# HazyResearch/hyena-dna

Measured on AMD Instinct MI355X. Metric: nucleotides/sec fwd+bwd at L=1M d=256; fftconv achieved HBM GB/s vs peak, higher is better.
Workload: dtype f32

## Files before the change

hyena_dna_amd/_lib.py:

```python
import ctypes
import os
import threading

import torch

HERE = os.path.dirname(os.path.abspath(__file__))
LIB_PATH = os.path.join(HERE, "csrc", "libhyena_fftconv.so")
ABI_VERSION = 3

HYENA_F32, HYENA_BF16, HYENA_F16 = 0, 1, 2
MAX_L = 1048576
PLAN_NONE, PLAN_ONCHIP, PLAN_TWO_LEVEL = 0, 1, 2

_DTYPES = {torch.float32: HYENA_F32, torch.bfloat16: HYENA_BF16, torch.float16: HYENA_F16}

_lock = threading.Lock()
_lib = None
_tables = {}
_workspace = {}


class HyenaLibraryError(RuntimeError):
    pass

# ... 110 lines not shown
                                        c_void_p]
        L.hyena_cm_post_bwd.restype = c_int
        L.hyena_cm_post_bwd.argtypes = [c_void_p, c_void_p, c_void_p, c_void_p, c_void_p, c_void_p, c_void_p, c_void_p, c_void_p,
                                        c_int, c_int, c_int, c_int, c_int, c_void_p]
        L.hyena_cm_pre_bwd.restype = c_int
        L.hyena_cm_pre_bwd.argtypes = [c_void_p, c_void_p, c_void_p, c_void_p, c_void_p, c_void_p, c_void_p,
                                       c_int, c_int, c_int, c_int, c_int, c_void_p]
        L.hyena_cm_pre_fwd_ld.restype = c_int
        L.hyena_cm_pre_fwd_ld.argtypes = [c_void_p, c_void_p, c_void_p, c_void_p, c_void_p, c_int, c_int, c_int, c_int, ctypes.c_long, c_int, c_int,
                                          c_int, c_void_p]
        L.hyena_cm_post_fwd_ld.restype = c_int
        L.hyena_cm_post_fwd_ld.argtypes = [c_void_p, c_void_p, c_void_p, c_void_p, c_void_p, c_void_p, c_int, c_int, c_int, c_int, ctypes.c_long, c_int,
                                           ctypes.c_long, c_int, c_int, c_int, c_void_p]
        L.hyena_cm_post_bwd_ld.restype = c_int
        L.hyena_cm_post_bwd_ld.argtypes = [c_void_p, c_void_p, c_void_p, c_void_p, c_void_p, c_void_p, c_void_p, c_void_p, c_void_p,
                                           c_int, c_int, c_int, c_int, ctypes.c_long, c_int, ctypes.c_long, c_int, c_int, c_int, c_void_p]
        L.hyena_cm_pre_bwd_ld.restype = c_int
        L.hyena_cm_pre_bwd_ld.argtypes = [c_void_p, c_void_p, c_void_p, c_void_p, c_void_p, c_void_p, c_void_p,
                                          c_int, c_int, c_int, c_int, ctypes.c_long, c_int, c_int, c_int, c_void_p]
        L.hyena_decode_partial_floats.restype = c_size_t
        L.hyena_decode_partial_floats.argtypes = [c_int, c_int, c_int]
        L.hyena_decode_pre.restype = c_int
        L.hyena_decode_pre.argtypes = [c_void_p, c_int, c_void_p, c_void_p, c_void_p, c_void_p, c_void_p, c_void_p, c_void_p,
                                       c_int, c_int, c_int, c_int, c_int, c_int, c_void_p]
        L.hyena_decode_conv.restype = c_int
        L.hyena_decode_conv.argtypes = [c_void_p, c_int, c_void_p, c_void_p, c_void_p, c_int, c_int, c_int, c_int, c_int, c_void_p]
        L.hyena_decode_post.restype = c_int
        L.hyena_decode_post.argtypes = [c_void_p, c_void_p, c_void_p, c_void_p, c_void_p, c_void_p, c_int, c_int, c_int, c_int, c_int, c_void_p]
        for rows, one in ((L.hyena_decode_pre_rows, L.hyena_decode_pre), (L.hyena_decode_conv_rows, L.hyena_decode_conv),
                          (L.hyena_decode_post_rows, L.hyena_decode_post)):
            rows.restype, rows.argtypes = c_int, one.argtypes
        L.hyena_decode_pre_fan.restype = c_int
        L.hyena_decode_pre_fan.argtypes = [c_void_p, c_int, c_void_p, c_void_p, c_void_p, c_void_p, c_void_p, c_void_p, c_void_p,
                                           c_int, c_int, c_int, c_int, c_int, c_int, c_int, c_void_p]
        L.hyena_decode_conv_fan.restype = c_int
        L.hyena_decode_conv_fan.argtypes = [c_void_p, c_int, c_void_p, c_void_p, c_void_p, c_void_p, c_int, c_int, c_int, c_int, c_int, c_int,
                                            c_int, c_int, c_void_p]
        L.hyena_decode_post_fan.restype = c_int
        L.hyena_decode_post_fan.argtypes = [c_void_p, c_void_p, c_void_p, c_void_p, c_void_p, c_void_p, c_int, c_int, c_int, c_int, c_int, c_int,
                                            c_int, c_void_p]
        L.hyena_decode_block_partial_floats.restype = c_size_t
        L.hyena_decode_block_partial_floats.argtypes = [c_int, c_int, c_int, c_int]
        for blk, one in ((L.hyena_decode_pre_block, L.hyena_decode_pre), (L.hyena_decode_conv_block, L.hyena_decode_conv),
                         (L.hyena_decode_post_block, L.hyena_decode_post), (L.hyena_decode_pre_block_fan, L.hyena_decode_pre_fan),
                         (L.hyena_decode_conv_block_fan, L.hyena_decode_conv_fan), (L.hyena_decode_post_block_fan, L.hyena_decode_post_fan)):
            blk.restype, blk.argtypes = c_int, one.argtypes[:-1] + [c_int, c_void_p]
        L.hyena_decode_sample.restype = c_int
        L.hyena_decode_sample.argtypes = [c_void_p, ctypes.c_long, c_int, c_int, c_int, c_int, ctypes.c_float, c_int, ctypes.c_float, c_void_p,
                                          c_int, c_int, c_void_p, c_void_p, c_void_p, ctypes.c_long, c_int, c_void_p, ctypes.c_long,
                                          c_void_p, c_void_p, c_void_p]
        L.hyena_inproj_pre_fwd_ld.restype = c_int
        L.hyena_inproj_pre_fwd_ld.argtypes = [c_void_p, c_void_p, c_void_p, c_void_p, c_void_p, c_void_p, c_void_p,
                                              c_int, c_int, c_int, c_int, ctypes.c_long, c_int, c_int, c_int, c_void_p]
        L.hyena_outproj_gate_addnorm_fwd_ld.restype = c_int
        L.hyena_outproj_gate_addnorm_fwd_ld.argtypes = [c_void_p, c_void_p, c_void_p, c_void_p, c_void_p, c_void_p, c_void_p, c_void_p, c_void_p,
                                                        c_void_p, ctypes.c_float, c_void_p, c_void_p, c_void_p, c_void_p, c_void_p,
                                                        c_int, c_int, c_int, c_int, ctypes.c_long, c_int, ctypes.c_long, c_int, c_int, c_int,
                                                        c_void_p]
        L.hyena_outproj_dgrad_supported.restype = c_int
        L.hyena_outproj_dgrad_supported.argtypes = [c_int, c_int, c_int, c_int]
        L.hyena_outproj_dgrad_partial_floats.restype = c_size_t
        L.hyena_outproj_dgrad_partial_floats.argtypes = [c_int, c_int, c_int]
        L.hyena_outproj_dgrad_gate_bwd_ld.restype = c_int
        L.hyena_outproj_dgrad_gate_bwd_ld.argtypes = [c_void_p, c_void_p, c_void_p, c_void_p, c_void_p, c_void_p, c_void_p, c_void_p, c_void_p,
                                                      c_void_p, c_int, c_int, c_int, c_int, ctypes.c_long, c_int, c_int, c_int, c_void_p]
        L.hyena_outproj_gate_fwd_ld.restype = c_int
        L.hyena_outproj_gate_fwd_ld.argtypes = [c_void_p, c_void_p, c_void_p, c_void_p, c_void_p, c_void_p, c_void_p, c_void_p, c_void_p,
                                                c_int, c_int, c_int, c_int, ctypes.c_long, c_int, ctypes.c_long, c_int, c_int, c_int, c_void_p]
        L.hyena_proj_supported.restype = c_int
        L.hyena_proj_supported.argtypes = [c_int, c_int, c_int, c_int]
        L.hyena_inproj_pre_fwd.restype = c_int
        L.hyena_inproj_pre_fwd.argtypes = [c_void_p, c_void_p, c_void_p, c_void_p, c_void_p, c_void_p, c_void_p,
                                           c_int, c_int, c_int, c_int, c_int, c_void_p]
        L.hyena_outproj_supported.restype = c_int
        L.hyena_outproj_supported.argtypes = [c_int, c_int, c_int, c_int]
        L.hyena_proj_kernel_generation.restype = c_int
        L.hyena_proj_kernel_generation.argtypes = [c_int, c_int]
        gen = os.environ.get("HYENA_OUTPROJ_KERNEL")
        if gen in ("1", "2"):
            L.hyena_proj_kernel_generation(0, int(gen))
        gen = os.environ.get("HYENA_INPROJ_KERNEL")
        if gen in ("1", "2"):
            L.hyena_proj_kernel_generation(1, int(gen))
        L.hyena_outproj_gate_fwd.restype = c_int
        L.hyena_outproj_gate_fwd.argtypes = [c_void_p, c_void_p, c_void_p, c_void_p, c_void_p, c_void_p, c_void_p, c_void_p, c_void_p,
                                             c_int, c_int, c_int, c_int, c_int, c_void_p]
        L.hyena_colsum_supported.restype = c_int
        L.hyena_colsum_supported.argtypes = [ctypes.c_long, c_int, c_int]
        L.hyena_colsum_partial_floats.restype = c_size_t
        L.hyena_colsum_partial_floats.argtypes = [ctypes.c_long, c_int]
        L.hyena_colsum.restype = c_int
        L.hyena_colsum.argtypes = [c_void_p, c_void_p, c_void_p, ctypes.c_long, c_int, c_int, c_void_p]
        L.hyena_mlp_supported.restype = c_int
        L.hyena_mlp_supported.argtypes = [ctypes.c_long, c_int, c_int, c_int]
        L.hyena_mlp_partial_floats.restype = c_size_t
        L.hyena_mlp_partial_floats.argtypes = [ctypes.c_long, c_int]
        L.hyena_mlp_fc1_gelu_fwd.restype = c_int
        L.hyena_mlp_fc1_gelu_fwd.argtypes = [c_void_p, c_void_p, c_void_p, c_void_p, c_void_p, ctypes.c_long, c_int, c_int, c_int, c_void_p]
        L.hyena_mlp_dh_dgelu_bwd.restype = c_int
        L.hyena_mlp_dh_dgelu_bwd.argtypes = [c_void_p, c_void_p, c_void_p, c_void_p, c_void_p, ctypes.c_long, c_int, c_int, c_int, c_void_p]
        L.hyena_filter_supported.restype = c_int
        L.hyena_filter_supported.argtypes = [c_int, c_int, c_int, c_int]
        L.hyena_filter_saved_bytes.restype = c_size_t
        L.hyena_filter_saved_bytes.argtypes = [c_int]
        L.hyena_filter_workspace_bytes.restype = c_size_t
        L.hyena_filter_workspace_bytes.argtypes = [c_int, c_int]
        L.hyena_filter_fwd.restype = c_int
        L.hyena_filter_fwd.argtypes = [ctypes.POINTER(FilterParams), c_void_p, c_void_p, c_void_p]
        L.hyena_filter_bwd.restype = c_int
        L.hyena_filter_bwd.argtypes = [ctypes.POINTER(FilterParams), c_void_p, c_void_p, ctypes.POINTER(FilterGrads),
                                       c_void_p, c_size_t, c_void_p]
        L.hyena_filter16_saved_bytes.restype = c_size_t
        L.hyena_filter16_saved_bytes.argtypes = [c_int]
        L.hyena_filter16_fwd.restype = c_int
        L.hyena_filter16_fwd.argtypes = [ctypes.POINTER(FilterParams), c_int, c_void_p, c_void_p, c_void_p]
        L.hyena_filter16_bwd.restype = c_int
        L.hyena_filter16_bwd.argtypes = [ctypes.POINTER(FilterParams), c_int, c_void_p, c_void_p, ctypes.POINTER(FilterGrads),
                                         c_void_p, c_size_t, c_void_p]
        L.hyena_filter_row_pitch.restype = c_int
        L.hyena_filter_row_pitch.argtypes = [c_int]
        L.hyena_filter_fwd_ld.restype = c_int
        L.hyena_filter_fwd_ld.argtypes = [ctypes.POINTER(FilterParams), c_void_p, c_int, c_void_p, c_void_p]
        L.hyena_filter_bwd_ld.restype = c_int
        L.hyena_filter_bwd_ld.argtypes = [ctypes.POINTER(FilterParams), c_void_p, c_int, c_void_p, ctypes.POINTER(FilterGrads),
                                          c_void_p, c_size_t, c_void_p]
        L.hyena_filter16_fwd_ld.restype = c_int
        L.hyena_filter16_fwd_ld.argtypes = [ctypes.POINTER(FilterParams), c_int, c_void_p, c_int, c_void_p, c_void_p]
        L.hyena_filter16_bwd_ld.restype = c_int
        L.hyena_filter16_bwd_ld.argtypes = [ctypes.POINTER(FilterParams), c_int, c_void_p, c_int, c_void_p, ctypes.POINTER(FilterGrads),
                                            c_void_p, c_size_t, c_void_p]
        c_long, c_float = ctypes.c_long, ctypes.c_float
        L.hyena_add_norm_supported.restype = c_int
        L.hyena_add_norm_supported.argtypes = [c_int, c_int, c_int]
        L.hyena_add_norm_fwd.restype = c_int
        L.hyena_add_norm_fwd.argtypes = [c_void_p, c_int, c_void_p, c_void_p, c_void_p, c_float, c_void_p, c_int, c_void_p,
                                         c_void_p, c_void_p, c_long, c_int, c_void_p]
        L.hyena_dropout_add_norm_fwd.restype = c_int
        L.hyena_dropout_add_norm_fwd.argtypes = [c_void_p, c_int, c_void_p, c_void_p, c_void_p, c_float, c_float, c_void_p, c_void_p, c_int,
                                                 c_void_p, c_void_p, c_void_p, c_long, c_int, c_void_p]
        L.hyena_dropout_add_norm_bwd.restype = c_int
        L.hyena_dropout_add_norm_bwd.argtypes = [c_void_p, c_int, c_void_p, c_void_p, c_void_p, c_void_p, c_void_p, c_float, c_void_p,
                                                 c_void_p, c_int, c_void_p, c_void_p, c_void_p, c_void_p, c_long, c_int, c_void_p]
        L.hyena_dropout_add_norm_bwd_colsum.restype = c_int
        L.hyena_dropout_add_norm_bwd_colsum.argtypes = [c_void_p, c_int, c_void_p, c_void_p, c_void_p, c_void_p, c_void_p, c_float, c_void_p,
                                                        c_void_p, c_int, c_void_p, c_void_p, c_void_p, c_void_p, c_void_p, c_long, c_int, c_void_p]
        L.hyena_embed_add_norm_supported.restype = c_int
        L.hyena_embed_add_norm_supported.argtypes = [c_int, c_int, c_int]
        L.hyena_embed_add_norm_fwd.restype = c_int
        L.hyena_embed_add_norm_fwd.argtypes = [c_void_p, c_void_p, c_int, c_void_p, c_void_p, c_float, c_float, c_void_p, c_void_p, c_int,
                                               c_void_p, c_void_p, c_void_p, c_long, c_int, c_void_p]
        L.hyena_embed_add_norm_partial_floats.restype = c_size_t
        L.hyena_embed_add_norm_partial_floats.argtypes = [c_long, c_int]
        L.hyena_embed_add_norm_bwd.restype = c_int
        L.hyena_embed_add_norm_bwd.argtypes = [c_void_p, c_int, c_void_p, c_void_p, c_void_p, c_void_p, c_void_p, c_void_p, c_float, c_void_p,
                                               c_void_p, c_int, c_void_p, c_void_p, c_void_p, c_long, c_int, c_void_p]
        L.hyena_add_norm_partial_floats.restype = c_size_t
        L.hyena_add_norm_partial_floats.argtypes = [c_long, c_int]
        L.hyena_add_norm_bwd.restype = c_int
        L.hyena_add_norm_bwd.argtypes = [c_void_p, c_int, c_void_p, c_void_p, c_void_p, c_void_p, c_void_p, c_void_p, c_int,
                                         c_void_p, c_void_p, c_void_p, c_void_p, c_long, c_int, c_void_p]
        L.hyena_add_norm_pool_supported.restype = c_int
        L.hyena_add_norm_pool_supported.argtypes = [c_int, c_int]
        L.hyena_add_norm_pool_partial_floats.restype = c_size_t
        L.hyena_add_norm_pool_partial_floats.argtypes = [c_int, c_long, c_int]
        L.hyena_add_norm_pool_fwd.restype = c_int
        L.hyena_add_norm_pool_fwd.argtypes = [c_void_p, c_int, c_void_p, c_void_p, c_void_p, c_float, c_float, c_void_p, c_void_p, c_int,
# ... 977 lines not shown
```

hyena_dna_amd/csrc/proj.hip:

```cpp
#include "proj_kernels.h"
#include "proj2_kernels.h"
#include "launch.h"
#include <type_traits>
#include "../../include/hyena_fftconv.h"
#include "../../include/hyena_proj.h"

using namespace hyena;

namespace {
template <auto Kernel, class Args>
int pj_launch(size_t lds, int threads, int grid, void* stream, const Args& a) {
    static thread_local int done = -1;
    hy_allow_lds(Kernel, lds, &done);
    HY_LAUNCH(Kernel, dim3(grid), dim3(threads), lds, stream, a);
    return hy_launch_error() ? HYENA_ERR_LAUNCH : HYENA_OK;
}
bool pj_kd_ok(int K, int dtype) { return (K == 128 || K == 256) && (dtype == HYENA_BF16 || dtype == HYENA_F16); }
template <class F>
int pj_dispatch(int K, int dtype, F f) {
    typedef std::integral_constant<int, DT_BF16> BF;
    typedef std::integral_constant<int, DT_F16> HF;
    if (K == 256) return dtype == HYENA_BF16 ? f(std::integral_constant<int, 256>(), BF()) : f(std::integral_constant<int, 256>(), HF());
    return dtype == HYENA_BF16 ? f(std::integral_constant<int, 128>(), BF()) : f(std::integral_constant<int, 128>(), HF());
}
int pj_runs(int tiles, int cap, int min_run, int* tiles_per_wg) {
    const int runs = cap < tiles ? cap : tiles;
    int len = (tiles + runs - 1) / runs;
    if (len < min_run && tiles >= min_run) len = min_run;
    *tiles_per_wg = len;
    return (tiles + len - 1) / len;
}
int pj_grid(int runs, int ncg) { return ((runs + 7) / 8) * 8 * ncg; }

void mlp_schedule(size_t P, int ncg, pj::MlpArgs* a, int* runs_out, int* grid_out) {
    a->tiles = (int)((P + pj::PJ_NT - 1) / pj::PJ_NT);
    *runs_out = pj_runs(a->tiles, 256 * 8 / ncg, 8, &a->tiles_per_wg);
    *grid_out = pj_grid(*runs_out, ncg);
}
void dgrad_schedule(int B, int L, int D, pj::DgArgs* a, int* runs_out, int* grid_out) {
    const int ncg = D / (pj::PJ_WAVES * pj::DG_CB);
    a->tiles_per_seq = (L + pj::PJ_NT - 1) / pj::PJ_NT;
    a->tiles = B * a->tiles_per_seq;
    a->nrec = *runs_out = pj_runs(a->tiles, 256 * DG_WGS / ncg, 16, &a->tiles_per_wg);
    *grid_out = pj_grid(*runs_out, ncg);
}
template <int MODE>
int dispatch_mlp(const pj::MlpArgs& a, int K, int dtype, int grid, void* stream) {
    return pj_dispatch(K, dtype, [&](auto k, auto dt) {
        constexpr int KK = decltype(k)::value, DT = decltype(dt)::value;
        return pj_launch<pj::mlp_kernel<KK, DT, MODE>>(pj::PmCfg<KK>::lds(MODE), pj::PJ_THREADS, grid, stream, a);
    });
}
int g_outproj_generation = 2;
int g_inproj_generation = 1;
}

#if defined(PJ_PROFILE)
extern "C" int hyena_pj_prof_set(void* buf) {
    return (int)hipMemcpyToSymbol(HIP_SYMBOL(hyena::pj::pj_prof_buf), &buf, sizeof(buf));
}
#endif

extern "C" {

static int colsum_groups(long P) {
    long g = (P + 511) / 512;
    return (int)(g < 1 ? 1 : (g > 512 ? 512 : g));
}

int hyena_colsum_supported(long P, int N, int dtype) {
    if (!(dtype == HYENA_BF16 || dtype == HYENA_F16) || N < 8 || N % 8 != 0 || pj::PJ_THREADS % (N / 8) != 0) return 0;
    return P >= 1 && (size_t)P < ((size_t)1 << 31) ? 1 : 0;
}

size_t hyena_colsum_partial_floats(long P, int N) { return P < 1 || N < 1 ? 0 : (size_t)colsum_groups(P) * N; }

int hyena_colsum(const void* x, float* part, float* out, long P, int N, int dtype, void* stream) {
    if (x == nullptr || part == nullptr || out == nullptr || !hyena_colsum_supported(P, N, dtype)) return HYENA_ERR_BAD_ARG;
    pj::ColsumArgs a;
    a.x = x; a.part = part; a.out = out; a.P = (unsigned)P; a.N = N; a.G = colsum_groups(P);
    a.rows_per_wg = (int)((P + a.G - 1) / a.G);
    a.G = (int)((P + a.rows_per_wg - 1) / a.rows_per_wg);
    const size_t lds = (size_t)pj::PJ_THREADS * 8 * sizeof(float);
    if (dtype == HYENA_BF16) HY_LAUNCH((pj::colsum_kernel<DT_BF16>), dim3(a.G), dim3(pj::PJ_THREADS), lds, stream, a);
    else HY_LAUNCH((pj::colsum_kernel<DT_F16>), dim3(a.G), dim3(pj::PJ_THREADS), lds, stream, a);
    HY_LAUNCH(pj::colsum_final_kernel, dim3((N + 63) / 64), dim3(pj::PJ_THREADS), pj::PJ_THREADS * sizeof(float), stream, a);
    return hy_launch_error() ? HYENA_ERR_LAUNCH : HYENA_OK;
}

int hyena_mlp_supported(long P, int K, int N, int dtype) {
    if (!pj_kd_ok(K, dtype)) return 0;
    if (N < 256 || N % 256 != 0 || P < 1) return 0;
    return (size_t)P < ((size_t)1 << 31) ? 1 : 0;
}

size_t hyena_mlp_partial_floats(long P, int N) {
    if (P < 1 || N < 256) return 0;
    pj::MlpArgs a;
    int runs, grid;
    mlp_schedule((size_t)P, N / 256, &a, &runs, &grid);
    return (size_t)runs * N;
}

int hyena_mlp_fc1_gelu_fwd(const void* x, const void* W1, const float* b1, void* a_out, void* h_out, long P, int K, int N, int dtype,
                           void* stream) {
    if (x == nullptr || W1 == nullptr || a_out == nullptr || h_out == nullptr || !hyena_mlp_supported(P, K, N, dtype)) return HYENA_ERR_BAD_ARG;
    pj::MlpArgs a;
    a.x = x; a.W = W1; a.bias = b1; a.a_in = nullptr; a.o0 = a_out; a.o1 = h_out; a.part = nullptr; a.P = (unsigned)P; a.N = N;
    int runs, grid;
    mlp_schedule((size_t)P, N / 256, &a, &runs, &grid);
    return dispatch_mlp<0>(a, K, dtype, grid, stream);
}

int hyena_mlp_dh_dgelu_bwd(const void* dy, const void* W2T, const void* a_in, void* da, float* part, long P, int K, int N, int dtype,
                           void* stream) {
    if (dy == nullptr || W2T == nullptr || a_in == nullptr || da == nullptr || part == nullptr || !hyena_mlp_supported(P, K, N, dtype))
        return HYENA_ERR_BAD_ARG;
    pj::MlpArgs a;
    a.x = dy; a.W = W2T; a.bias = nullptr; a.a_in = a_in; a.o0 = da; a.o1 = nullptr; a.part = part; a.P = (unsigned)P; a.N = N;
    int runs, grid;
    mlp_schedule((size_t)P, N / 256, &a, &runs, &grid);
    return dispatch_mlp<1>(a, K, dtype, grid, stream);
}

int hyena_proj_kernel_generation(int family, int generation) {
    if (family != 0 && family != 1) return -1;
    int& g = family == 0 ? g_outproj_generation : g_inproj_generation;
    if (generation == 1 || generation == 2) g = generation;
    else if (generation > 0) return -1;
    return g;
}

int hyena_outproj_supported(int B, int L, int D, int dtype) {
    if (!pj_kd_ok(D, dtype)) return 0;
    if (B < 1 || L < 64) return 0;
    return (size_t)B * (size_t)L < ((size_t)1 << 31) ? 1 : 0;
}

int hyena_outproj_gate_fwd(const void* y, const void* xT, const float* bin, const float* w, const float* b, const void* W,
                           const float* bias, void* out, void* zT, int B, int L, int Lx, int D, int dtype, void* stream) {
    return hyena_outproj_gate_fwd_ld(y, xT, bin, w, b, W, bias, out, zT, B, L, Lx, D, (long)B * Lx, Lx, (long)B * L, L, L, dtype, stream);
}

int hyena_outproj_gate_fwd_ld(const void* y, const void* xT, const float* bin, const float* w, const float* b, const void* W,
                              const float* bias, void* out, void* zT, int B, int L, int Lx, int D, long csx, int bsx, long csz, int bsz,
                              int lda, int dtype, void* stream) {
    return hyena_outproj_gate_addnorm_fwd_ld(y, xT, bin, w, b, W, bias, nullptr, nullptr, nullptr, 0.f, out, nullptr, nullptr, nullptr, zT, B, L,
                                             Lx, D, csx, bsx, csz, bsz, lda, dtype, stream);
}

static bool pj_layout_ok(long cs, int bs, int B, int len) { return bs >= len && cs >= (long)(B - 1) * bs + len; }

int hyena_outproj_gate_addnorm_fwd_ld(const void* y, const void* xT, const float* bin, const float* w, const float* b, const void* W,
                                      const float* bias, const float* residual_in, const float* ln_weight, const float* ln_bias, float eps,
                                      void* out, float* residual_out, float* mean, float* rstd, void* zT, int B, int L, int Lx, int D,
                                      long csx, int bsx, long csz, int bsz, int lda, int dtype, void* stream) {
    if (y == nullptr || xT == nullptr || w == nullptr || b == nullptr || W == nullptr || out == nullptr || L > Lx || lda < L ||
        !hyena_outproj_supported(B, L, D, dtype) || !pj_layout_ok(csx, bsx, B, Lx) || (zT != nullptr && !pj_layout_ok(csz, bsz, B, L)))
        return HYENA_ERR_BAD_ARG;
    if (ln_weight != nullptr && (ln_bias == nullptr || residual_out == nullptr || mean == nullptr || rstd == nullptr ||
                                 residual_out == residual_in))
        return HYENA_ERR_BAD_ARG;
    pj::OutProjArgs a;
    a.y = y; a.xT = xT; a.bin = bin; a.w = w; a.b = b; a.W = W; a.bias = bias; a.out = out; a.zT = zT;
    a.res_in = residual_in; a.ln_w = ln_weight; a.ln_b = ln_bias; a.res_out = residual_out; a.mean = mean; a.rstd = rstd; a.eps = eps;
    a.B = B; a.L = L; a.Lx = Lx; a.D = D; a.csx = csx; a.bsx = bsx; a.csz = csz; a.bsz = bsz; a.lda = lda;
    a.tiles_per_seq = (L + pj::PJ_NT - 1) / pj::PJ_NT;
    a.tiles = B * a.tiles_per_seq;
    const bool gen2 = g_outproj_generation == 2;
    const bool ln = ln_weight != nullptr;
    const int runs = pj_runs(a.tiles, 256 * (gen2 && D == 256 ? 4 : 8), 8, &a.tiles_per_wg);
    return pj_dispatch(D, dtype, [&](auto k, auto dt) {
        constexpr int K = decltype(k)::value, DT = decltype(dt)::value;
        typedef pj::Op2Cfg<K> C2;
        typedef pj::OpCfg<K> C1;
        if (gen2)
            return ln ? pj_launch<pj::outproj_gate_fwd2_kernel<K, DT, true>>(C2::LDS_LN, C2::THREADS, runs, stream, a)
                      : pj_launch<pj::outproj_gate_fwd2_kernel<K, DT, false>>(C2::LDS, C2::THREADS, runs, stream, a);
        return ln ? pj_launch<pj::outproj_gate_fwd_kernel<K, DT, true>>(C1::LDS_LN, pj::PJ_THREADS, runs, stream, a)
                  : pj_launch<pj::outproj_gate_fwd_kernel<K, DT, false>>(C1::LDS, pj::PJ_THREADS, runs, stream, a);
    });
}

int hyena_outproj_dgrad_supported(int B, int L, int D, int dtype) {
    if (!pj_kd_ok(D, dtype)) return 0;
    if (B < 1 || L < 1) return 0;
    return (size_t)B * (size_t)L < ((size_t)1 << 31) - 64 ? 1 : 0;
}

size_t hyena_outproj_dgrad_partial_floats(int B, int L, int D) {
    if (B < 1 || L < 1 || !(D == 128 || D == 256)) return 0;
    pj::DgArgs a;
    int runs, grid;
    dgrad_schedule(B, L, D, &a, &runs, &grid);
    return (size_t)D * runs * 8;
}

int hyena_outproj_dgrad_gate_bwd_ld(const void* dy, const void* Wt, const void* y, const void* xT, const float* bin, const float* w,
                                    const float* b, void* dyc, void* dxT, float* part, int B, int L, int Lx, int D, long csx, int bsx,
                                    int lda, int dtype, void* stream) {
    if (dy == nullptr || Wt == nullptr || y == nullptr || xT == nullptr || w == nullptr || b == nullptr || dyc == nullptr || dxT == nullptr ||
        part == nullptr || L > Lx || !pj_layout_ok(csx, bsx, B, Lx) || lda < L || !hyena_outproj_dgrad_supported(B, L, D, dtype))
        return HYENA_ERR_BAD_ARG;
    pj::DgArgs a;
    a.dy = dy; a.Wt = Wt; a.y = y; a.xT = xT; a.bin = bin; a.w = w; a.b = b; a.dyc = dyc; a.dxT = dxT; a.part = part;
    a.B = B; a.L = L; a.Lx = Lx; a.D = D; a.csx = csx; a.bsx = bsx; a.lda = lda;
    int runs, grid;
    dgrad_schedule(B, L, D, &a, &runs, &grid);
    return pj_dispatch(D, dtype, [&](auto k, auto dt) {
        constexpr int K = decltype(k)::value, DT = decltype(dt)::value;
// ... 49 lines not shown
```

hyena_dna_amd/csrc/proj2_kernels.h:

```cpp
#pragma once
#include "proj_kernels.h"

namespace hyena {
namespace pj {

template <int K> struct Op2Cfg {
    static_assert(K == 128 || K == 256, "d_model of the HyenaDNA models");
    static constexpr int WAVES = K / 16;
    static constexpr int THREADS = WAVES * 64;
    static constexpr int KS = K / 32;
    static constexpr int RND = K / (WAVES * 8);
    static constexpr int ZBUF = PJ_NT * K * 2;
    static constexpr int TAPB = K * 8 * 4;
    static constexpr int OROW = (K + 8) * 2;
    static constexpr int OBUF = PJ_NT * OROW;
    static constexpr int ROWS = PJ_NT / WAVES;
    static constexpr size_t LDS = (size_t)ZBUF + TAPB + OBUF;
    static constexpr int RROW = K * 4;
    static constexpr int RBUF = PJ_NT * RROW;
    static constexpr size_t LDS_LN = LDS + RBUF;
};

template <int K, int DT, bool LN>
__global__ void __launch_bounds__(Op2Cfg<K>::THREADS, 4) outproj_gate_fwd2_kernel(OutProjArgs a) {
// ... 456 lines not shown
                vg_half(0, 0, prod);
                vg_half(0, 1, prod);
                vg_store(0, prod);
            } else {
                product(0, Q);
                HY_SCHED_FENCE();
                xt_load();
                HY_SCHED_FENCE();
                product(Q, 2 * Q);
                HY_SCHED_FENCE();
                xt_store(0, 2);
                HY_SCHED_FENCE();
                product(2 * Q, 3 * Q);
                HY_SCHED_FENCE();
                xt_store(2, 4);
                HY_SCHED_FENCE();
                product(3 * Q, 4 * Q);
                HY_SCHED_FENCE();
                vg_half(0, 0, prod);
                HY_SCHED_FENCE();
                product(4 * Q, 5 * Q);
                HY_SCHED_FENCE();
                vg_half(0, 1, prod);
                vg_store(0, prod);
                HY_SCHED_FENCE();
                product(5 * Q, 6 * Q);
                HY_SCHED_FENCE();
                if (nunits > 1) vg_half(1, 0, prod);
                HY_SCHED_FENCE();
                product(6 * Q, 7 * Q);
                HY_SCHED_FENCE();
                if (nunits > 1) { vg_half(1, 1, prod); vg_store(1, prod); }
                HY_SCHED_FENCE();
                product(7 * Q, C::KS);
            }
        } else {
            if (pend) row_phase_generic();
            product(0, C::KS);
        }
        PJ_MARK(3);
        PJ_BARRIER();
        PJ_MARK(4);
        if (have) {
            if (lane < IP2_CB) {
                HY_LDS uint32_t* row = reinterpret_cast<HY_LDS uint32_t*>(et + (lr0 + lane) * C::EROW);
                row[3] = row[3 + PJ_NT / 2];
            }
            HY_WAVE_SYNC_PJ();
            HY_UNROLL
            for (int pt = 0; pt < 2; ++pt) {
                elem_t e16[16];
                HY_UNROLL
                for (int r = 0; r < 16; ++r) e16[r] = Elem<DT>::cvt(acc[pt][r]);
                Frag f0, f1;
                __builtin_memcpy(f0.w, e16, 16);
                __builtin_memcpy(f1.w, e16 + 8, 16);
                HY_LDS char* dst = et + (lr0 + j) * C::EROW + (8 + 32 * pt + 16 * hb) * 2;
                lds_st16(dst, f0);
                lds_st16(dst + 16, f1);
            }
        }
        pend = have && t >= t_begin;
        pend_fast = p0 + PJ_NT <= P && sl0 >= 2 && sl0 + PJ_NT <= a.Lc;
        prev_p0 = p0; prev_sb = sb; prev_sl0 = sl0;
        PJ_MARK(5);
    }
#if defined(PJ_PROFILE) && !defined(HIPEMU)
    asm volatile("s_waitcnt vmcnt(0)" ::: "memory");
    PJ_MARK(9);
    asm volatile("s_memrealtime %0\n\ts_waitcnt lgkmcnt(0)" : "=s"(pj_rt1)::"memory");
    if (pj_prof_buf != nullptr && lane == 0) {
        unsigned long long* o = pj_prof_buf + ((size_t)blockIdx.x * IP2_WAVES + wave) * 16;
        HY_UNROLL
        for (int i = 0; i < 10; ++i) o[i] = pj_d[i];
        o[10] = (unsigned long long)(t_end - t_first + 1);
        o[11] = pj_t - pj_start;
        o[12] = pj_rt1 - pj_rt0;
    }
#endif
}

}
}
```

hyena_dna_amd/csrc/proj_kernels.h:

```cpp
#pragma once
#define HY_HELPERS_ONLY
#include "fftconv_kernels.h"
#include "block_kernels.h"

namespace hyena {
namespace pj {

enum { PJ_THREADS = 256, PJ_WAVES = 4, PJ_NT = 64 ,
       PJ_EW = PJ_NT + 8  };

#ifdef HIPEMU
#define HY_WAVE_SYNC_PJ() hipemu::yield(2)
#else
#define HY_WAVE_SYNC_PJ() __builtin_amdgcn_wave_barrier()
#endif

#if defined(PJ_PROFILE) && !defined(HIPEMU)
__device__ unsigned long long* pj_prof_buf = nullptr;
#define PJ_NOW(v)                                                                                       \
    do {                                                                                                \
        __builtin_amdgcn_sched_barrier(0);                                                              \
        asm volatile("s_memtime %0\n\ts_waitcnt lgkmcnt(0)" : "=s"(v)::"memory");                       \
        __builtin_amdgcn_sched_barrier(0);                                                              \
    } while (0)
// ... 24 lines not shown
        return __builtin_amdgcn_mfma_f32_32x32x16_f16(__builtin_bit_cast(v8, a), __builtin_bit_cast(v8, b), c, 0, 0, 0);
    }
}
#endif

#ifdef HIPEMU
__device__ __forceinline__ Frag ld16(const void* p) { Frag f; __builtin_memcpy(f.w, p, 16); return f; }
__device__ __forceinline__ void st16(void* p, const Frag& f) { __builtin_memcpy(p, f.w, 16); }
__device__ __forceinline__ Frag lds_ld16(const HY_LDS char* p) { return ld16(p); }
__device__ __forceinline__ void lds_st16(HY_LDS char* p, const Frag& f) { st16(p, f); }
#else
typedef unsigned pj_vec16 __attribute__((ext_vector_type(4), aligned(2)));
typedef unsigned pj_lvec16 __attribute__((ext_vector_type(4)));
__device__ __forceinline__ Frag ld16(const void* p) {
#ifdef PJ_DBG_NO_LD
    Frag f; f.w[0] = f.w[1] = f.w[2] = f.w[3] = (uint32_t)(size_t)p; return f;
#else
    return __builtin_bit_cast(Frag, *reinterpret_cast<const pj_vec16*>(p));
#endif
}
#ifndef PJ_POL_ST
#define PJ_POL_ST 1
#endif
__device__ __forceinline__ void st16(void* p, const Frag& f) {
#ifdef PJ_DBG_NO_ST
    if (f.w[0] == 0x12345678u && f.w[3] == 0x9abcdef0u) *reinterpret_cast<pj_vec16*>(p) = __builtin_bit_cast(pj_vec16, f);
#else
    if (PJ_POL_ST) __builtin_nontemporal_store(__builtin_bit_cast(pj_vec16, f), reinterpret_cast<pj_vec16*>(p));
    else *reinterpret_cast<pj_vec16*>(p) = __builtin_bit_cast(pj_vec16, f);
#endif
}
__device__ __forceinline__ Frag lds_ld16(const HY_LDS char* p) { return __builtin_bit_cast(Frag, *reinterpret_cast<const HY_LDS pj_lvec16*>(p)); }
__device__ __forceinline__ void lds_st16(HY_LDS char* p, const Frag& f) { *reinterpret_cast<HY_LDS pj_lvec16*>(p) = __builtin_bit_cast(pj_lvec16, f); }
#endif

#ifdef HIPEMU
struct EmuVmq {
    struct Op { const void* src; void* dst; };
    Op q[128];
    int head = 0, n = 0;
    void push(const void* src, void* dst) { q[(head + n++) & 127] = Op{src, dst}; }
    void retire_to(int keep) {
        while (n > keep) {
            const Op& o = q[head];
            if (o.dst != nullptr) __builtin_memcpy(o.dst, o.src, 16);
            head = (head + 1) & 127;
            --n;
        }
    }
    ~EmuVmq() { retire_to(0); }
};
#define PJ_VMQ_DECL EmuVmq pj_vmq
#define PJ_VMQ_PARAM , EmuVmq& pj_vmq
#define PJ_VMQ_ARG , pj_vmq
__device__ __forceinline__ void glds16(const char* base, uint32_t voff, HY_LDS char* wave_base, int lane, EmuVmq& q) { q.push(base + voff, wave_base + 16 * lane); }
#define PJ_VMWAIT(n) pj_vmq.retire_to(n)
#define PJ_LGKMWAIT() do {} while (0)
#define PJ_BARRIER() __syncthreads()
#define PJ_ST16(p, f) do { st16((p), (f)); pj_vmq.push(nullptr, nullptr); } while (0)
#else
#define PJ_VMQ_DECL do {} while (0)
#define PJ_VMQ_PARAM
#define PJ_VMQ_ARG
#define PJ_ST16(p, f) st16((p), (f))
#pragma clang diagnostic push
#pragma clang diagnostic ignored "-Winline-asm"
__device__ __forceinline__ void glds16(const char* base, uint32_t voff, HY_LDS char* wave_base, int lane) {
    (void)lane;
#ifdef PJ_DBG_NO_LD
    return;
#endif
    asm volatile("s_mov_b32 m0, %2\n\ts_nop 0\n\tglobal_load_lds_dwordx4 %0, %1"
                 :: "v"(voff), "s"(base), "s"((uint32_t)(size_t)wave_base) : "memory", "m0");
}
#pragma clang diagnostic pop
#define PJ_VMWAIT(n) asm volatile("s_waitcnt vmcnt(" #n ")" ::: "memory")
#define PJ_LGKMWAIT() asm volatile("s_waitcnt lgkmcnt(0)" ::: "memory")
#define PJ_BARRIER() do { asm volatile("s_waitcnt lgkmcnt(0)" ::: "memory"); __builtin_amdgcn_s_barrier(); } while (0)
#endif

struct True_ { static constexpr bool value = true; };
struct False_ { static constexpr bool value = false; };

template <int K, bool FULL>
__device__ __forceinline__ void issue_operand_tile(const char* xbase, unsigned p0, unsigned P, HY_LDS char* ubuf, int wave, int lane PJ_VMQ_PARAM) {
    constexpr int PCS = K / 8, NX = PJ_NT * K * 2 / 1024 / PJ_WAVES;
    const char* const tb = HY_UNIFORM_PTR(const char, xbase + (size_t)p0 * K * 2);
    HY_OPAQUE(lane);
    HY_UNROLL
    for (int i = 0; i < NX; ++i) {
        const int chunk = i * PJ_WAVES + wave, S = chunk * 64 + lane, pos = S / PCS, c = (S % PCS) ^ (pos % PCS);
        if (FULL || p0 + (unsigned)pos < P) glds16(tb, (uint32_t)(pos * K * 2 + c * 16), ubuf + chunk * 1024, lane PJ_VMQ_ARG);
    }
}

template <int K> struct PjCfg {
    static_assert(K == 128 || K == 256, "d_model of the HyenaDNA models");
    static constexpr int KS = K / 16;
    static constexpr int UROW = (K + 8) * 2;
    static constexpr int UBUF = PJ_NT * UROW;
    static constexpr int CH = PJ_NT * K * 2 / 16 / PJ_THREADS;
};

struct InProjArgs {
    const void* u;
    const void* W;
    const float* bin;
    const float* w;
    const float* b;
    void* xT;
    void* vg;
    int B, Lx, Lc, D;
    long csx; int bsx;
    int ldv;
    int tiles;
    int tiles_per_wg;
};

__device__ __forceinline__ int pj_row(int r, int hb) { return (r & 3) + 8 * (r >> 2) + 4 * hb; }

#ifdef HIPEMU
typedef hipemu::floatx4 acc4_t;
template <int DT>
__device__ __forceinline__ acc4_t mfma16(const Frag& a, const Frag& b, acc4_t c) {
    hipemu::u32x4 x, y;
    __builtin_memcpy(x.w, a.w, 16);
    __builtin_memcpy(y.w, b.w, 16);
    return hipemu::mfma_f32_16x16x32_h<DT == DT_BF16>(x, y, c);
}
#else
typedef float acc4_t __attribute__((ext_vector_type(4)));
template <int DT>
__device__ __forceinline__ acc4_t mfma16(const Frag& a, const Frag& b, acc4_t c) {
    if constexpr (DT == DT_BF16) {
        typedef __bf16 v8 __attribute__((ext_vector_type(8)));
        return __builtin_amdgcn_mfma_f32_16x16x32_bf16(__builtin_bit_cast(v8, a), __builtin_bit_cast(v8, b), c, 0, 0, 0);
    } else {
        typedef _Float16 v8 __attribute__((ext_vector_type(8)));
        return __builtin_amdgcn_mfma_f32_16x16x32_f16(__builtin_bit_cast(v8, a), __builtin_bit_cast(v8, b), c, 0, 0, 0);
    }
}
#endif

enum { IP_CB = 16, IP_NT4 = PJ_NT / 16 };
template <int K> struct IpCfg {
    static constexpr int KS = K / 32;
    static constexpr int PCS = K / 8;
    static constexpr int UROWB = K * 2, UBUF = PJ_NT * UROWB;
    static constexpr int EROW = PJ_EW * 2;
    static constexpr int EBUF = 3 * IP_CB * EROW;
    static constexpr int TAPS = 2 * IP_CB * 5 * 4;
    static constexpr size_t LDS = (size_t)UBUF + PJ_WAVES * ((size_t)EBUF + TAPS);
};

template <int K, int DT>
__global__ void __launch_bounds__(PJ_THREADS, 2) inproj_pre_fwd_kernel(InProjArgs a) {
    typedef IpCfg<K> C;
    typedef typename Elem<DT>::type elem_t;
    static_assert(sizeof(elem_t) == 2, "16-bit element types only");
    HY_SMEM(smem);
    PJ_VMQ_DECL;
    const int tid = (int)threadIdx.x, wave = HY_SGPR(tid >> 6), lane = tid & 63, j = lane & 15, kq = lane >> 4;
    const int D = a.D;
    const unsigned P = (unsigned)a.B * (unsigned)a.Lx;
    const int ncg = D / (PJ_WAVES * IP_CB);
    int cg, run;
    {
        const int wg = blockIdx.x, xcd = wg & 7, seq = wg >> 3;
        cg = seq % ncg;
        run = (seq / ncg) * 8 + xcd;
    }
    const int t_begin = run * a.tiles_per_wg;
    if (t_begin >= a.tiles) return;
    const int t_end = (t_begin + a.tiles_per_wg < a.tiles) ? t_begin + a.tiles_per_wg : a.tiles;
// ... 1030 lines not shown
```

Measured before the change: 164.6 million.

## Add 8-wave MLP kernel generation and default backward dgelu to it

Adds a second-generation MLP projection kernel with 8 waves per workgroup. Each wave holds a 32-column weight slice in registers. The result tile goes through an LDS image so global stores are coalesced, and the activation operand for the backward pass is streamed through per-wave LDS slots. The backward (MODE 1) path now defaults to the new kernel while the forward stays on generation 1, and an env var can select either. This is meant to improve HBM streaming efficiency of the dh/dgelu pass, but it uses more LDS and a different grid mapping, which may reduce occupancy.

After: 164.7 million, median of 4. About the same (+0.0%).

```diff
diff --git a/hyena_dna_amd/_lib.py b/hyena_dna_amd/_lib.py
--- a/hyena_dna_amd/_lib.py
+++ b/hyena_dna_amd/_lib.py
@@ -216,6 +216,10 @@
         gen = os.environ.get("HYENA_INPROJ_KERNEL")
         if gen in ("1", "2"):
             L.hyena_proj_kernel_generation(1, int(gen))
+        gen = os.environ.get("HYENA_MLP_KERNEL")
+        if gen in ("1", "2"):
+            L.hyena_proj_kernel_generation(2, int(gen))
+            L.hyena_proj_kernel_generation(3, int(gen))
         L.hyena_outproj_gate_fwd.restype = c_int
         L.hyena_outproj_gate_fwd.argtypes = [c_void_p, c_void_p, c_void_p, c_void_p, c_void_p, c_void_p, c_void_p, c_void_p, c_void_p,
                                              c_int, c_int, c_int, c_int, c_int, c_void_p]
diff --git a/hyena_dna_amd/csrc/proj.hip b/hyena_dna_amd/csrc/proj.hip
--- a/hyena_dna_amd/csrc/proj.hip
+++ b/hyena_dna_amd/csrc/proj.hip
@@ -44,15 +44,18 @@
     a->nrec = *runs_out = pj_runs(a->tiles, 256 * DG_WGS / ncg, 16, &a->tiles_per_wg);
     *grid_out = pj_grid(*runs_out, ncg);
 }
+int g_outproj_generation = 2;
+int g_inproj_generation = 1;
+int g_mlp_generation[2] = {1, 2};
 template <int MODE>
 int dispatch_mlp(const pj::MlpArgs& a, int K, int dtype, int grid, void* stream) {
+    const bool gen2 = g_mlp_generation[MODE] == 2;
     return pj_dispatch(K, dtype, [&](auto k, auto dt) {
         constexpr int KK = decltype(k)::value, DT = decltype(dt)::value;
+        if (gen2) return pj_launch<pj::mlp2_kernel<KK, DT, MODE>>(pj::Pm2Cfg<KK>::lds(MODE), pj::PM2_THREADS, grid, stream, a);
         return pj_launch<pj::mlp_kernel<KK, DT, MODE>>(pj::PmCfg<KK>::lds(MODE), pj::PJ_THREADS, grid, stream, a);
     });
 }
-int g_outproj_generation = 2;
-int g_inproj_generation = 1;
 }
 
 #if defined(PJ_PROFILE)
@@ -124,8 +127,8 @@
 }
 
 int hyena_proj_kernel_generation(int family, int generation) {
-    if (family != 0 && family != 1) return -1;
-    int& g = family == 0 ? g_outproj_generation : g_inproj_generation;
+    if (family < 0 || family > 3) return -1;
+    int& g = family == 0 ? g_outproj_generation : family == 1 ? g_inproj_generation : g_mlp_generation[family - 2];
     if (generation == 1 || generation == 2) g = generation;
     else if (generation > 0) return -1;
     return g;
diff --git a/hyena_dna_amd/csrc/proj2_kernels.h b/hyena_dna_amd/csrc/proj2_kernels.h
--- a/hyena_dna_amd/csrc/proj2_kernels.h
+++ b/hyena_dna_amd/csrc/proj2_kernels.h
@@ -562,3 +562,210 @@
 
 }
 }
+
+namespace hyena {
+namespace pj {
+
+enum { PM2_WAVES = 8, PM2_THREADS = PM2_WAVES * 64, PM2_UW = 32 , PM2_STEPS = PJ_NT / PM2_WAVES / 2  };
+template <int K> struct Pm2Cfg {
+    static_assert(K == 128 || K == 256, "d_model of the HyenaDNA models");
+    static constexpr int KS = K / 16;
+    static constexpr int PCS = K / 8;
+    static constexpr int UROWB = K * 2;
+    static constexpr int UBUF = PJ_NT * UROWB;
+    static constexpr int NX = UBUF / 1024 / PM2_WAVES;
+    static constexpr int IROW = PM2_WAVES * PM2_UW * 2;
+    static constexpr int IMG = PJ_NT * IROW;
+    static constexpr int ASLOTS = 2 * 1024;
+    static constexpr size_t lds(int mode) { return (size_t)UBUF + IMG + (mode == 0 ? 0 : PM2_WAVES * ASLOTS); }
+};
+
+template <int K, int DT, int MODE>
+__global__ void __launch_bounds__(PM2_THREADS, 4) mlp2_kernel(MlpArgs a) {
+    typedef Pm2Cfg<K> C;
+    typedef typename Elem<DT>::type elem_t;
+    static_assert(sizeof(elem_t) == 2, "16-bit element types only");
+    HY_SMEM(smem);
+    PJ_VMQ_DECL;
+    const int tid = (int)threadIdx.x, wave = HY_SGPR(tid >> 6), lane = tid & 63, j = lane & 31, hb = lane >> 5;
+    const int N = a.N;
+    const unsigned P = a.P;
+    const int ncg = N / (PM2_WAVES * PM2_UW);
+    int cg, run;
+    {
+        const int wg = blockIdx.x, xcd = wg & 7, seq = wg >> 3;
+        cg = seq % ncg;
+        run = (seq / ncg) * 8 + xcd;
+    }
+    const int t_begin = run * a.tiles_per_wg;
+    if (t_begin >= a.tiles) return;
+    const int t_end = (t_begin + a.tiles_per_wg < a.tiles) ? t_begin + a.tiles_per_wg : a.tiles;
+    const int nw = cg * PM2_WAVES * PM2_UW, n0 = nw + wave * PM2_UW;
+
+    HY_LDS char* const ubuf = HY_LDS_CAST(char, smem);
+    HY_LDS char* const img = HY_LDS_CAST(char, smem) + C::UBUF;
+    HY_LDS char* const aslot = HY_LDS_CAST(char, smem) + C::UBUF + C::IMG + wave * C::ASLOTS;
+
+    const char* const xbase = reinterpret_cast<const char*>(a.x);
+    auto issue_x = [&](int t, auto full_c) {
+        issue_operand_tile<K, decltype(full_c)::value, PM2_WAVES>(xbase, (unsigned)t * PJ_NT, P, ubuf, wave, lane PJ_VMQ_ARG);
+    };
+    const int rrow = wave * 8 + 4 * hb, pcs = j ^ (hb << 2);
+    const uint32_t goff0 = (uint32_t)((rrow * N + nw + 8 * pcs) * 2);
+    auto issue_a = [&](int t, int m, auto full_c) {
+        constexpr bool FULL = decltype(full_c)::value;
+        const unsigned p0 = (unsigned)t * PJ_NT;
+        const char* const rb = HY_UNIFORM_PTR(const char, reinterpret_cast<const char*>(a.a_in) + ((size_t)p0 + (unsigned)m) * N * 2);
+        if (FULL || p0 + (unsigned)(rrow + m) < P) glds16(rb, goff0, aslot + (m & 1) * 1024, lane PJ_VMQ_ARG);
+    };
+    const int t_whole = (int)(P / PJ_NT) < t_end ? (int)(P / PJ_NT) : t_end;
+    if (t_begin < t_whole) { issue_x(t_begin, True_()); if (MODE == 1) { issue_a(t_begin, 0, True_()); issue_a(t_begin, 1, True_()); } }
+    else { issue_x(t_begin, False_()); if (MODE == 1) { issue_a(t_begin, 0, False_()); issue_a(t_begin, 1, False_()); } }
+
+    Frag wf[C::KS];
+    {
+        const char* row = reinterpret_cast<const char*>(a.W) + ((size_t)(n0 + j) * K + 8 * hb) * 2;
+        HY_UNROLL
+        for (int ks = 0; ks < C::KS; ++ks) wf[ks] = ld16(row + ks * 32);
+    }
+    float bias = MODE == 0 && a.bias != nullptr ? a.bias[n0 + j] : 0.f;
+    HY_UNROLL
+    for (int ks = 0; ks < C::KS; ++ks) HY_OPAQUE(wf[ks].w[0]);
+    HY_OPAQUE(bias);
+    float colsum[8] = {0.f, 0.f, 0.f, 0.f, 0.f, 0.f, 0.f, 0.f};
+
+    const int ua = j * C::UROWB, ux = (hb ^ (j % C::PCS)) * 16;
+    HY_LDS char* const pk = img + (4 * hb) * C::IROW + ((wave * 4 + (j >> 3)) ^ (hb << 2)) * 16 + (j & 7) * 2;
+    const HY_LDS char* const rd = img + rrow * C::IROW + j * 16;
+
+#if defined(PJ_PROFILE) && !defined(HIPEMU)
+    unsigned long long pj_d[12] = {0, 0, 0, 0, 0, 0, 0, 0, 0, 0, 0, 0}, pj_t, pj_start, pj_rt0, pj_rt1;
+    asm volatile("s_memrealtime %0\n\ts_waitcnt lgkmcnt(0)" : "=s"(pj_rt0)::"memory");
+    PJ_NOW(pj_t);
+    pj_start = pj_t;
+#endif
+    auto tile = [&](int t, auto full_c, auto next_c) {
+        constexpr bool full = decltype(full_c)::value, next_full = decltype(next_c)::value;
+        const unsigned p0 = (unsigned)t * PJ_NT;
+        if (t == t_begin || !full) PJ_VMWAIT(0);
+        else PJ_VMWAIT(8);
+        PJ_MARK(0);
+        PJ_BARRIER();
+        PJ_MARK(1);
+        acc_t acc[2];
+        HY_UNROLL
+        for (int pt = 0; pt < 2; ++pt) {
+            HY_UNROLL
+            for (int r = 0; r < 16; ++r) acc[pt][r] = 0.f;
+        }
+        HY_UNROLL
+        for (int ks = 0; ks < C::KS; ++ks) {
+            HY_UNROLL
+            for (int pt = 0; pt < 2; ++pt) {
+                const Frag af = lds_ld16(ubuf + pt * 32 * C::UROWB + ua + (ux ^ (ks * 32)));
+                acc[pt] = mfma<DT>(af, wf[ks], acc[pt]);
+            }
+        }
+        PJ_MARK(2);
+        HY_UNROLL
+        for (int pt = 0; pt < 2; ++pt) {
+            HY_UNROLL
+            for (int r = 0; r < 16; ++r) {
+                const float v = acc[pt][r];
+                *reinterpret_cast<HY_LDS elem_t*>(pk + (32 * pt + (r & 3) + 8 * (r >> 2)) * C::IROW) = Elem<DT>::cvt(MODE == 0 ? v + bias : v);
+            }
+        }
+        PJ_BARRIER();
+        PJ_MARK(3);
+        if (next_full) issue_x(t + 1, True_());
+        else if (t + 1 < t_end) issue_x(t + 1, False_());
+        PJ_MARK(4);
+        char* const dst0 = reinterpret_cast<char*>(a.o0) + (size_t)p0 * N * 2 + goff0;
+        char* const dst1 = MODE == 0 ? reinterpret_cast<char*>(a.o1) + (size_t)p0 * N * 2 + goff0 : nullptr;
+        Frag rp[PM2_STEPS];
+        if (MODE == 0) {
+            HY_UNROLL
+            for (int m = 0; m < PM2_STEPS; ++m) rp[m] = lds_ld16(rd + m * C::IROW);
+        }
+        HY_UNROLL
+        for (int m = 0; m < PM2_STEPS; ++m) {
+            const bool on = full || p0 + (unsigned)(rrow + m) < P;
+            elem_t ge[8], oe[8];
+            if (MODE == 0) {
+                __builtin_memcpy(ge, rp[m].w, 16);
+                HY_UNROLL
+                for (int i = 0; i < 8; ++i) oe[i] = Elem<DT>::cvt(pm_gelu(Elem<DT>::dec(ge[i])));
+                Frag rh;
+                __builtin_memcpy(rh.w, oe, 16);
+                if (on) {
+                    PJ_ST16(dst0 + (size_t)m * N * 2, rp[m]);
+                    PJ_ST16(dst1 + (size_t)m * N * 2, rh);
+                }
+            } else {
+                if (!full || !next_full) PJ_VMWAIT(0);
+                else if (m >= 2) PJ_VMWAIT(3);
+                else if (C::NX == 4) PJ_VMWAIT(7);
+                else PJ_VMWAIT(5);
+                rp[m] = lds_ld16(rd + m * C::IROW);
+                const Frag af = lds_ld16(aslot + (m & 1) * 1024 + lane * 16);
+                PJ_LGKMWAIT();
+                if (m + 2 < PM2_STEPS) issue_a(t, m + 2, full_c);
+                else if (next_full) issue_a(t + 1, m + 2 - PM2_STEPS, True_());
+                else if (t + 1 < t_end) issue_a(t + 1, m + 2 - PM2_STEPS, False_());
+                elem_t ae[8];
+                __builtin_memcpy(ge, rp[m].w, 16);
+                __builtin_memcpy(ae, af.w, 16);
+                Frag rdv;
+                HY_UNROLL
+                for (int i = 0; i < 8; ++i) {
+                    oe[i] = Elem<DT>::cvt(Elem<DT>::dec(ge[i]) * pm_dgelu(Elem<DT>::dec(ae[i])));
+                    if (on) colsum[i] += Elem<DT>::dec(oe[i]);
+                    if (i & 1) rdv.w[i >> 1] = (uint32_t)oe[i - 1] | ((uint32_t)oe[i] << 16);
+                    if (i == 3) HY_SCHED_FENCE();
+                }
+                if (on) PJ_ST16(dst0 + (size_t)m * N * 2, rdv);
+            }
+        }
+        PJ_MARK(5);
+    };
+    {
+        int t = t_begin;
+        for (; t + 1 < t_whole; ++t) tile(t, True_(), True_());
+        if (t < t_whole) { tile(t, True_(), False_()); ++t; }
+        if (t < t_end) tile(t, False_(), False_());
+    }
+#if defined(PJ_PROFILE) && !defined(HIPEMU)
+    asm volatile("s_waitcnt vmcnt(0)" ::: "memory");
+    PJ_MARK(9);
+    asm volatile("s_memrealtime %0\n\ts_waitcnt lgkmcnt(0)" : "=s"(pj_rt1)::"memory");
+    if (pj_prof_buf != nullptr && lane == 0) {
+        unsigned long long* o = pj_prof_buf + ((size_t)blockIdx.x * PM2_WAVES + wave) * 16;
+        HY_UNROLL
+        for (int i = 0; i < 10; ++i) o[i] = pj_d[i];
+        o[10] = (unsigned long long)(t_end - t_begin);
+        o[11] = pj_t - pj_start;
+        o[12] = pj_rt1 - pj_rt0;
+        unsigned hw, xcc;
+        asm volatile("s_getreg_b32 %0, hwreg(HW_REG_HW_ID)" : "=s"(hw));
+        asm volatile("s_getreg_b32 %0, hwreg(HW_REG_XCC_ID)" : "=s"(xcc));
+        o[13] = ((unsigned long long)xcc << 32) | hw;
+        o[14] = pj_start;
+    }
+#endif
+    if (MODE == 1) {
+        HY_LDS float* red = reinterpret_cast<HY_LDS float*>(img);
+        PJ_BARRIER();
+        HY_UNROLL
+        for (int i = 0; i < 8; ++i) red[(wave * 2 + hb) * (PM2_WAVES * PM2_UW) + 8 * pcs + i] = colsum[i];
+        PJ_BARRIER();
+        if (tid < PM2_WAVES * PM2_UW) {
+            float sum = 0.f;
+            HY_UNROLL
+            for (int w = 0; w < PM2_WAVES; ++w) sum += red[(2 * w) * (PM2_WAVES * PM2_UW) + tid] + red[(2 * w + 1) * (PM2_WAVES * PM2_UW) + tid];
+            a.part[(size_t)run * N + nw + tid] = sum;
+        }
+    }
+}
+
+}
+}
diff --git a/hyena_dna_amd/csrc/proj_kernels.h b/hyena_dna_amd/csrc/proj_kernels.h
--- a/hyena_dna_amd/csrc/proj_kernels.h
+++ b/hyena_dna_amd/csrc/proj_kernels.h
@@ -130,14 +130,14 @@
 struct True_ { static constexpr bool value = true; };
 struct False_ { static constexpr bool value = false; };
 
-template <int K, bool FULL>
+template <int K, bool FULL, int WAVES = PJ_WAVES>
 __device__ __forceinline__ void issue_operand_tile(const char* xbase, unsigned p0, unsigned P, HY_LDS char* ubuf, int wave, int lane PJ_VMQ_PARAM) {
-    constexpr int PCS = K / 8, NX = PJ_NT * K * 2 / 1024 / PJ_WAVES;
+    constexpr int PCS = K / 8, NX = PJ_NT * K * 2 / 1024 / WAVES;
     const char* const tb = HY_UNIFORM_PTR(const char, xbase + (size_t)p0 * K * 2);
     HY_OPAQUE(lane);
     HY_UNROLL
     for (int i = 0; i < NX; ++i) {
-        const int chunk = i * PJ_WAVES + wave, S = chunk * 64 + lane, pos = S / PCS, c = (S % PCS) ^ (pos % PCS);
+        const int chunk = i * WAVES + wave, S = chunk * 64 + lane, pos = S / PCS, c = (S % PCS) ^ (pos % PCS);
         if (FULL || p0 + (unsigned)pos < P) glds16(tb, (uint32_t)(pos * K * 2 + c * 16), ubuf + chunk * 1024, lane PJ_VMQ_ARG);
     }
 }
```
